# zssjh/stereo-semantic-vo

Measured on AMD Instinct MI355X. Metric: stereo frames/sec on KITTI 00 (full Tracking::Track chain), higher is better.
Workload: dtype u8; 1 GPU; BASELINE configs[2]: synth-kitti00 sequence of 4541 distinct 1241x376 stereo pairs, full Tracking::Track loop per frame (ORB on L and R, sparse stereo, matching passes 1+2, PnP-RANSAC, pose-only LM, map-point lifecycle); ONE sequence per GPU in strict frame order (replicas across GPUs); parallelism=one GPU, resident_pairs_per_gpu=4541, resident_input_bytes_per_gpu=4370984960, frames_tracked=4541, tracker_capacity_flag=0, pnp_samples_through_sequential_fallback=0

## Files before the change

stereo-semantic-vo_amd/csrc/svo_epnp_ord_dev.h:

```cpp
#pragma once
#ifndef HIP_INCLUDE_HIP_HIP_RUNTIME_H
#include <hip/hip_runtime.h>
#endif
#include <stdint.h>

#include "svo_epnp_exact_dev.h"

namespace epnp_ord {

#define EO_FN __device__ __forceinline__
typedef double d2 __attribute__((ext_vector_type(2)));

#include "svo_epnp_ord_tab.h"
#include "svo_epnp_ord_asm.h"

#define EO_SYNC()                                         \
  do {                                                    \
    __builtin_amdgcn_fence(__ATOMIC_ACQ_REL, "wavefront"); \
    __builtin_amdgcn_wave_barrier();                      \
  } while (0)

struct Lds {
  alignas(16) double jr[16 * 16];
  alignas(16) double xch[16][4][4];
  unsigned tab[EO_TAB_TOTAL];
  double pws[16], us[10], alphas[20], cws[12], ccinv[9];
  double M[120];
  double ut4[4][12];
  double L[60], rho[6];
  double sw[3][6];
  double bx[3][6];
  double ccs[3][12], pcs[3][16], abt[3][9], Rc[3][9], rep[3][8];
  alignas(16) double gn[3][6][6];
  double out[3][16];
  int srow[3][6];
  int urow[4];
  double xw[16];
  int flag;
  int sweeps;
  int why;
  long long stamp[8];
#ifdef EO_PROFILE
  long long prof[8];
#endif
};

EO_FN double xdiv(double a, double b) { return a / b; }
EO_FN double xsqrt(double x) { return sqrt(x); }

EO_FN double ndiv(double a, double b) {
  double r = __builtin_amdgcn_rcp(b);
  double e = __builtin_fma(-b, r, 1.0);
  r = __builtin_fma(r, e, r);
  e = __builtin_fma(-b, r, 1.0);
  r = __builtin_fma(r, e, r);
  const double q = a * r;
  const double rem = __builtin_fma(-b, q, a);
  return __builtin_fma(rem, r, q);
}
EO_FN double nsqrt(double x) {
  const double y = __builtin_amdgcn_rsq(x);
  double g = x * y, h = 0.5 * y;
  const double r = __builtin_fma(-h, g, 0.5);
  g = __builtin_fma(g, r, g);
  h = __builtin_fma(h, r, h);
  double d = __builtin_fma(-g, g, x);
  g = __builtin_fma(d, h, g);
  d = __builtin_fma(-g, g, x);
  g = __builtin_fma(d, h, g);
  return g;
}
EO_FN bool w_in_range(double w) { return w >= 7.888609052210118e-31 && w <= 1.2676506002282294e30; }

EO_FN double gsum(double term, double acc) { return __builtin_amdgcn_mfma_f64_4x4x4f64(1.0, term, acc, 0, 0, 0); }
template <int M>
EO_FN double colsum(double t0, double t1, double t2, int g) {
  double acc = gsum(M >= 4 || g < M ? t0 : 0.0, 0.0);
  if (M > 4) acc = gsum(M >= 8 || 4 + g < M ? t1 : 0.0, acc);
  if (M > 8) acc = gsum(M >= 12 || 8 + g < M ? t2 : 0.0, acc);
  return acc;
}

#define EO_TAB3_OFF 0
#define EO_TAB4_OFF (EO_TAB3_OFF + EO_TAB3_STEPS * 3)
#define EO_TAB5_OFF (EO_TAB4_OFF + EO_TAB4_STEPS * 4)
#define EO_TAB12_OFF (EO_TAB5_OFF + EO_TAB5_STEPS * 5)
EO_FN unsigned tab_entry(unsigned e) { return (e & ~16u) | ((e & 16u) << 27); }
EO_FN void load_tables(Lds& S, int lane) {
  for (int e = lane; e < EO_TAB3_STEPS * 3; e += 64) S.tab[EO_TAB3_OFF + e] = tab_entry(c_tab3[0][e]);
  for (int e = lane; e < EO_TAB4_STEPS * 4; e += 64) S.tab[EO_TAB4_OFF + e] = tab_entry(c_tab4[0][e]);
  for (int e = lane; e < EO_TAB5_STEPS * 5; e += 64) S.tab[EO_TAB5_OFF + e] = tab_entry(c_tab5[0][e]);
  for (int e = lane; e < EO_TAB12_STEPS * 12; e += 64) S.tab[EO_TAB12_OFF + e] = tab_entry(c_tab12[0][e]);
}

// ... 357 lines not shown
      double eta = fabs(A[k][k]);
#pragma unroll
      for (int i = k + 1; i < 6; ++i) {
        const double elt = fabs(A[i - 1][k]);
        if (eta < elt) eta = elt;
      }
      if (eta == 0) alive = false;
      const double inv_eta = 1. / eta;
      double sum2 = 0.0;
#pragma unroll
      for (int i = k; i < 6; ++i) {
        A[i][k] *= inv_eta;
        sum2 += A[i][k] * A[i][k];
      }
      double sigma = xsqrt(sum2);
      if (A[k][k] < 0) sigma = -sigma;
      A[k][k] += sigma;
      A1[k] = sigma * A[k][k];
      A2[k] = -eta * sigma;
#pragma unroll
      for (int j = k + 1; j < 4; ++j) {
        double sum = 0;
#pragma unroll
        for (int i = k; i < 6; ++i) sum += A[i][k] * A[i][j];
        const double tau = sum / A1[k];
#pragma unroll
        for (int i = k; i < 6; ++i) A[i][j] -= tau * A[i][k];
      }
    }
#pragma unroll
    for (int j = 0; j < 4; ++j) {
      double tau = 0;
#pragma unroll
      for (int i = j; i < 6; ++i) tau += A[i][j] * b[i];
      tau /= A1[j];
#pragma unroll
      for (int i = j; i < 6; ++i) b[i] -= tau * A[i][j];
    }
    x[3] = b[3] / A2[3];
#pragma unroll
    for (int i = 2; i >= 0; --i) {
      double sum = 0;
#pragma unroll
      for (int j = i + 1; j < 4; ++j) sum += A[i][j] * x[j];
      x[i] = (b[i] - sum) / A2[i];
    }
#pragma unroll
    for (int i = 0; i < 4; ++i) betas[i] += alive ? x[i] : 0.0;
  }
}

EO_FN double dot3(const double* a, const double* b) { return a[0] * b[0] + a[1] * b[1] + a[2] * b[2]; }

EO_FN bool solve5_wave(Lds& S, epnp_exact::Work& xw, const double* K, double* R_out, double* t_out, double* rep, bool force_seq = false) {
  const int lane = threadIdx.x & 63, slot = lane >> 4, col = lane & 15, r16 = lane & 15;
  const double fu = K[0], fv = K[1], uc = K[2], vc = K[3];
  if (lane == 0) { S.flag = force_seq ? 1 : 0; S.why = force_seq ? 16 : 0; S.stamp[0] = clock64(); }
  load_tables(S, lane);
  EO_SYNC();
  if (lane < 3) {
    double c = 0;
    for (int i = 0; i < 5; i++) c += S.pws[3 * i + lane];
    S.cws[lane] = c / 5;
  }
  EO_SYNC();
  auto load_pw0 = [&]() {
    if (lane < 9) {
      const int a = lane / 3, b = lane % 3;
      const double ca = S.cws[a], cb = S.cws[b];
      double s = 0;
      for (int i = 0; i < 5; ++i) s += (S.pws[3 * i + a] - ca) * (S.pws[3 * i + b] - cb);
      S.jr[b * 16 + a] = s;
    } else if (lane < 18) {
      const int r = (lane - 9) / 3, k = (lane - 9) % 3;
      S.jr[r * 16 + 3 + k] = r == k ? 1.0 : 0.0;
    } else if (lane < 36) {
      S.jr[((lane - 18) / 6) * 16 + 6 + (lane - 18) % 6] = 0.0;
    }
    EO_SYNC();
  };
  load_pw0();
  unsigned long long ex = jacobi_rows<3>(S, r16 < 3 ? 3 : 0, r16 < 3 ? 0 : r16, lane);
  unsigned long long bd = svd_rank(S, slot == 0 ? 3 : 0, 0, 0, lane);
  if (ex | bd) {
    load_pw0();
    if (lane == 0) svd_small_seq(S, xw.jW, 3, 3, 0, 0);
    EO_SYNC();
  }
  if (lane < 9) {
    const int i = 1 + lane / 3, j = lane % 3;
    const double k = xsqrt(S.sw[0][i - 1] / 5);
    S.cws[3 * i + j] = S.cws[j] + k * S.jr[S.srow[0][i - 1] * 16 + j];
  }
  EO_SYNC();
  auto load_cc = [&]() {
    if (lane < 9) {
      const int r = lane / 3, k = lane % 3;
      S.jr[r * 16 + k] = S.cws[3 * (r + 1) + k] - S.cws[k];
    } else if (lane < 18) {
      const int r = (lane - 9) / 3, k = (lane - 9) % 3;
      S.jr[r * 16 + 3 + k] = r == k ? 1.0 : 0.0;
    } else if (lane < 36) {
      S.jr[((lane - 18) / 6) * 16 + 6 + (lane - 18) % 6] = 0.0;
    }
    EO_SYNC();
  };
  load_cc();
  ex = jacobi_rows<3>(S, r16 < 3 ? 3 : 0, r16 < 3 ? 0 : r16, lane);
  bd = svd_rank(S, slot == 0 ? 3 : 0, 0, 0, lane);
  if (ex | bd) {
    load_cc();
    if (lane == 0) svd_small_seq(S, xw.jW, 3, 3, 0, 0);
// ... 271 lines not shown
```

stereo-semantic-vo_amd/csrc/svo_pose_dev.h:

```cpp
#pragma once
#include "svo_internal.h"
#include "svo_wave.h"

struct Se3 { double q[4]; double t[3]; };

__device__ __forceinline__ double pose_ndiv(double a, double b) {
  double r = __builtin_amdgcn_rcp(b);
  double e = __builtin_fma(-b, r, 1.0);
  r = __builtin_fma(r, e, r);
  e = __builtin_fma(-b, r, 1.0);
  r = __builtin_fma(r, e, r);
  const double q = a * r;
  const double rem = __builtin_fma(-b, q, a);
  return __builtin_fma(rem, r, q);
}
__device__ __forceinline__ double pose_rcp_refined(double b) {
  double r = __builtin_amdgcn_rcp(b);
  double e = __builtin_fma(-b, r, 1.0);
  r = __builtin_fma(r, e, r);
  e = __builtin_fma(-b, r, 1.0);
  r = __builtin_fma(r, e, r);
  return r;
}
__device__ __forceinline__ double pose_ndiv_r(double a, double b, double r) {
// ... 327 lines not shown

__device__ __forceinline__ void pose_edge_regs(const double* Xw, const double* obs, int n, double first[10], int sx = 3, int so = 2) {
  const int lane = threadIdx.x & 63, a = min(lane, n - 1), b = min(64 + lane, n - 1);
  first[0] = Xw[sx * a]; first[1] = Xw[sx * a + 1]; first[2] = Xw[sx * a + 2]; first[3] = obs[so * a]; first[4] = obs[so * a + 1];
  first[5] = Xw[sx * b]; first[6] = Xw[sx * b + 1]; first[7] = Xw[sx * b + 2]; first[8] = obs[so * b]; first[9] = obs[so * b + 1];
}

__device__ __forceinline__ void build_system_ordered(const Se3& est, const double* Xw, const double* obs, int n, const double* K,
                                                     double delta, double dsqr, double* tw_all , double* red,
                                                     bool on_mfma, const double first[10]) {
  const int tid = threadIdx.x, lane = tid & 63, wv = __builtin_amdgcn_readfirstlane(tid >> 6);
  const int g = lane >> 4, c = lane & 15;
  double* tw = tw_all + wv * POSE_CHUNK * POSE_TW;
  double acc = 0.0;
  for (int e0 = 0; e0 < n; e0 += POSE_CHUNK) {
    const int cnt = min(POSE_CHUNK, n - e0);
    if (cnt > 64) {
      switch (wv) {
        case 0: wave_terms_to_lds<0, true>(est, Xw, obs, n, e0, lane, K, delta, dsqr, tw, first); break;
        case 1: wave_terms_to_lds<1, true>(est, Xw, obs, n, e0, lane, K, delta, dsqr, tw, first); break;
        case 2: wave_terms_to_lds<2, true>(est, Xw, obs, n, e0, lane, K, delta, dsqr, tw, first); break;
        default: wave_terms_to_lds<3, true>(est, Xw, obs, n, e0, lane, K, delta, dsqr, tw, first); break;
      }
    } else {
      switch (wv) {
        case 0: wave_terms_to_lds<0, false>(est, Xw, obs, n, e0, lane, K, delta, dsqr, tw, first); break;
        case 1: wave_terms_to_lds<1, false>(est, Xw, obs, n, e0, lane, K, delta, dsqr, tw, first); break;
        case 2: wave_terms_to_lds<2, false>(est, Xw, obs, n, e0, lane, K, delta, dsqr, tw, first); break;
        default: wave_terms_to_lds<3, false>(est, Xw, obs, n, e0, lane, K, delta, dsqr, tw, first); break;
      }
    }
    POSE_WSYNC();
    if (on_mfma) acc = pose_chain_sum(tw + min(c, POSE_TW - 1), POSE_TW, cnt, g, acc);
    else acc = pose_lane_sum(tw + min(lane, POSE_QW - 1), POSE_TW, cnt, acc);
    POSE_WSYNC();
  }
  if (lane < POSE_QW) red[wv * POSE_QW + lane] = acc;
  __syncthreads();
}

__device__ __forceinline__ void unpack_system(const double* red, double H[36], double b[6]) {
  int k = 0;
#pragma unroll
  for (int r = 0; r < 6; ++r)
#pragma unroll
    for (int c = r; c < 6; ++c) { H[6 * r + c] = red[k]; H[6 * c + r] = red[k]; ++k; }
#pragma unroll
  for (int r = 0; r < 6; ++r) b[r] = red[21 + r];
}

struct LmShared {
  Se3 est;
  int go;
  int done;
};

#define PNP_HYP 100
#define PNP_MAXN 512

struct PoseLds {
  double tw[4 * POSE_CHUNK * POSE_TW];
  double red[POSE_NQ + 4];
  LmShared sh;
  double K[4];
};

__device__ __forceinline__ void build_system_one_lane(const Se3& est, const double* Xw, const double* obs, int n, const double* K,
                                                      double delta, double dsqr, double* red) {
  if (threadIdx.x == 0) {
    double acc[POSE_NQ];
    for (int k = 0; k < POSE_NQ; ++k) acc[k] = 0.0;
    for (int i = 0; i < n; ++i) {
      double e[2], pc[3], J[12], rz;
      edge_error(est, Xw + 3 * i, obs + 2 * i, K, e, pc, &rz);
      double rho0 = e[0] * e[0] + e[1] * e[1], rho1 = 1.;
      huber(rho0, delta, dsqr, rho0, rho1);
      edge_jacobian(pc, K, J, rz);
      int k = 0;
      for (int r = 0; r < 6; ++r)
        for (int c = r; c < 6; ++c) acc[k++] += rho1 * (J[r] * J[c] + J[6 + r] * J[6 + c]);
      for (int r = 0; r < 6; ++r) acc[21 + r] -= rho1 * (J[r] * e[0] + J[6 + r] * e[1]);
      acc[27] += rho0;
    }
    for (int k = 0; k < POSE_NQ; ++k) red[k] = acc[k];
  }
  __syncthreads();
}

struct PosePrepared { const Se3* est; const double* first; };
__device__ __forceinline__ void pose_start_estimate(const double* T, int round_in_f32, Se3& est0) {
  if (round_in_f32) {
    double Tf[16];
    for (int j = 0; j < 16; ++j) Tf[j] = (double)(float)T[j];
    se3_from_T(Tf, est0);
  } else {
    se3_from_T(T, est0);
  }
}

template <int NT = 256>
__device__ __forceinline__ void pose_opt_block(PoseLds& L, const double* __restrict__ Xw, const double* __restrict__ obs, int n,
                                               const double* __restrict__ Kp, double* T, svo_lm_stats* stats,
                                               int round_in_f32, int use_ordered_mfma, long long* t_first_build = nullptr,
                                               const PosePrepared* prep = nullptr, double* T_lds = nullptr, int* iters_out = nullptr) {
  static_assert(NT == 256, "pose_opt_block: four waves (wave w owns the quantities 7 w .. 7 w + 6 of the normal equations)");
  double* red = L.red; LmShared& sh = L.sh; double* K = L.K;
  const int tid = threadIdx.x;
  const double delta = (double)(float)sqrt(5.991);
  const double dsqr = delta * delta;
  Se3 est0{};
  double first[10];
  if (prep && prep->est) {
    if (tid == 0) { est0 = *prep->est; sh.est = est0; sh.done = 0; }
#pragma unroll
    for (int k = 0; k < 10; ++k) first[k] = prep->first[k];
  } else {
    __syncthreads();
    if (!prep && tid < 4) K[tid] = Kp[tid];
    if (tid == 0) {
      pose_start_estimate(T, round_in_f32, est0);
      sh.est = est0;
      sh.done = 0;
    }
    if (prep) {
#pragma unroll
      for (int k = 0; k < 10; ++k) first[k] = prep->first[k];
    } else if (n > 0) {
      pose_edge_regs(Xw, obs, n, first);
    }
  }
  __syncthreads();
  double lambda = -1., ni = 2., currentChi = 0, chi_init = 0;
  int nBad = 0, iters = 0, trials_total = 0, terminated = 0;
  if (n <= 0) {
    if (tid == 0 && stats) {
      stats->n_edges = 0; stats->iterations = 0; stats->trials_total = 0; stats->terminated = 0;
      stats->chi2_initial = 0; stats->chi2_final = 0; stats->lambda_final = 0;
    }
    if (tid == 0 && T_lds)
      for (int j = 0; j < 16; ++j) T_lds[j] = T[j];
    if (tid == 0 && iters_out) *iters_out = 0;
    return;
  }
#ifdef POSE_PROF
  long long pf_build = 0, pf_serial = 0, pf_dec = 0, pf_t = 0;
#define PF(acc) do { const long long _n = clock64(); acc += _n - pf_t; pf_t = _n; } while (0)
  pf_t = clock64();
#else
#define PF(acc) do { } while (0)
#endif
  auto build = [&]() {
    const Se3 est = sh.est;
    if (use_ordered_mfma) build_system_ordered(est, Xw, obs, n, K, delta, dsqr, L.tw, red, use_ordered_mfma == 1, first);
    else build_system_one_lane(est, Xw, obs, n, K, delta, dsqr, red);
  };
  if (t_first_build && tid == 0) *t_first_build = wall_clock64();
  build();
  PF(pf_build);
  double H[36], b[6], x[6] = {0, 0, 0, 0, 0, 0};
  if (tid == 0) {
    unpack_system(red, H, b);
    currentChi = red[27];
    chi_init = currentChi;
    double maxDiag = 0;
    for (int j = 0; j < 6; ++j) maxDiag = fmax(fabs(H[7 * j]), maxDiag);
    lambda = 1e-5 * maxDiag;
  }
  for (int it = 0; it < 10; ++it) {
    double iniChi = currentChi, rho = 0;
    int qmax = 0;
    for (int trial = 0; trial < 10; ++trial) {
      int ok2 = 0;
      if (tid == 0) {
        double Hl[36];
#pragma unroll
        for (int j = 0; j < 36; ++j) Hl[j] = H[j];
#pragma unroll
        for (int j = 0; j < 6; ++j) Hl[7 * j] += lambda;
        ok2 = ldlt6_solve(Hl, b, x);
        Se3 e2 = est0;
        se3_oplus(x, e2);
        sh.est = e2;
      }
      __syncthreads();
      PF(pf_serial);
      build();
      PF(pf_build);
      if (tid == 0) {
        double tempChi = red[27];
        if (!ok2) tempChi = 1.7976931348623157e308;
        rho = currentChi - tempChi;
        double scale = 0;
        for (int j = 0; j < 6; ++j) scale += x[j] * (lambda * x[j] + b[j]);
        scale += 1e-3;
        rho /= scale;
        if (rho > 0 && isfinite(tempChi)) {
          const double v = 2 * rho - 1;
          double alpha = 1. - v * v * v;
          alpha = fmin(alpha, 2. / 3.);
          const double scaleFactor = fmax(1. / 3., alpha);
          lambda *= scaleFactor;
          ni = 2;
          currentChi = tempChi;
          est0 = sh.est;
          unpack_system(red, H, b);
        } else {
          lambda *= ni;
          ni *= 2;
        }
        ++qmax;
        ++trials_total;
        sh.go = (rho < 0 && qmax < 10) ? 1 : 0;
      }
      __syncthreads();
      PF(pf_dec);
      if (!sh.go) break;
    }
    if (tid == 0) {
      ++iters;
      int stop = 0;
      if (qmax == 10 || rho == 0) stop = 1;
      else {
        if ((iniChi - currentChi) * 1e3 < iniChi) ++nBad; else nBad = 0;
        if (nBad >= 3) stop = 1;
      }
      if (stop) terminated = 1;
      sh.done = stop;
    }
    __syncthreads();
    if (sh.done) break;
  }
  if (tid == 0) {
    se3_to_T(est0, T);
    if (T_lds) se3_to_T(est0, T_lds);
    if (iters_out) *iters_out = iters;
    if (stats) {
      stats->n_edges = n; stats->iterations = iters; stats->trials_total = trials_total;
      stats->terminated = terminated; stats->chi2_initial = chi_init;
      stats->chi2_final = currentChi; stats->lambda_final = lambda;
#ifdef POSE_PROF
      stats->chi2_initial = (double)pf_build; stats->chi2_final = (double)pf_serial; stats->lambda_final = (double)pf_dec;
#endif
    }
  }
}

#include "svo_epnp_dev.h"
#include "svo_epnp_exact_dev.h"
#include "svo_epnp_ord_dev.h"

struct PnpHyp {
  double R[9], t[3];
  int32_t cnt, ok;
};

__device__ __forceinline__ bool pnp_inlier(const double* R, const double* t, const double* X, const double* uv, const double* K) {
  double x = R[0] * X[0] + R[1] * X[1] + R[2] * X[2] + t[0];
  double y = R[3] * X[0] + R[4] * X[1] + R[5] * X[2] + t[1];
  double z = R[6] * X[0] + R[7] * X[1] + R[8] * X[2] + t[2];
  z = z != 0.0 ? 1. / z : 1.;
  x *= z; y *= z;
  const float px = (float)(x * K[0] + K[2]), py = (float)(y * K[1] + K[3]);
  const float dx = (float)uv[0] - px, dy = (float)uv[1] - py;
  const float err = dx * dx + dy * dy;
  return err <= 64.0f;
}

__device__ __forceinline__ void pnp_hyp_block(EpnpWaveLds* ws, const double* Xw, const double* uv, int n, const double* K,
                                              const uint16_t* subset, PnpHyp* out, int hyp_base) {
  const int lane = threadIdx.x & 63, wv = threadIdx.x >> 6;
  const int k = hyp_base + wv;
  if (k >= PNP_HYP) return;
  if (lane < 5) {
    const int e = min((int)subset[5 * k + lane], n - 1);
    ws[wv].x5[3 * lane] = Xw[3 * e]; ws[wv].x5[3 * lane + 1] = Xw[3 * e + 1]; ws[wv].x5[3 * lane + 2] = Xw[3 * e + 2];
    ws[wv].u5[2 * lane] = uv[2 * e]; ws[wv].u5[2 * lane + 1] = uv[2 * e + 1];
  }
  double R[9], t[3];
  const bool ok = epnp5_wave(ws[wv], K, R, t);
  int cnt = 0;
  if (ok)
    for (int e = lane; e < n; e += 64) cnt += pnp_inlier(R, t, Xw + 3 * e, uv + 2 * e, K) ? 1 : 0;
  cnt = wave_sum_i32_dpp(cnt);
  if (lane == 0) {
    PnpHyp h;
#pragma unroll
    for (int i = 0; i < 9; ++i) h.R[i] = R[i];
    h.t[0] = t[0]; h.t[1] = t[1]; h.t[2] = t[2];
    h.cnt = cnt; h.ok = ok ? 1 : 0;
    out[k] = h;
  }
}

struct PnpExactLds { epnp_exact::Work W; double R[9], t[3]; int ok; };
__device__ __forceinline__ void pnp_hyp_exact_wave(PnpExactLds& S, const double* Xw, const double* uv, int n, const double* K,
                                                   const uint16_t* subset, PnpHyp* out, int k) {
  const int lane = threadIdx.x & 63;
  if (k >= PNP_HYP) return;
  if (lane == 0) {
    double* x5 = S.W.PW0;
    double* u5 = S.W.gA;
    for (int i = 0; i < 5; ++i) {
      const int e = min((int)subset[5 * k + i], n - 1);
      x5[3 * i] = Xw[3 * e]; x5[3 * i + 1] = Xw[3 * e + 1]; x5[3 * i + 2] = Xw[3 * e + 2];
      u5[2 * i] = uv[2 * e]; u5[2 * i + 1] = uv[2 * e + 1];
    }
    S.ok = epnp_exact::solve5(S.W, x5, u5, K, S.R, S.t, nullptr) ? 1 : 0;
  }
  __builtin_amdgcn_fence(__ATOMIC_ACQ_REL, "workgroup");
  __builtin_amdgcn_wave_barrier();
  double R[9], t[3];
#pragma unroll
  for (int i = 0; i < 9; ++i) R[i] = S.R[i];
#pragma unroll
  for (int i = 0; i < 3; ++i) t[i] = S.t[i];
  const bool ok = S.ok != 0;
  int cnt = 0;
  if (ok)
    for (int e = lane; e < n; e += 64) cnt += pnp_inlier(R, t, Xw + 3 * e, uv + 2 * e, K) ? 1 : 0;
  cnt = wave_sum_i32_dpp(cnt);
  if (lane == 0) {
    PnpHyp h;
#pragma unroll
    for (int i = 0; i < 9; ++i) h.R[i] = R[i];
    h.t[0] = t[0]; h.t[1] = t[1]; h.t[2] = t[2];
    h.cnt = cnt; h.ok = ok ? 1 : 0;
    out[k] = h;
  }
}

struct PnpOrdLds { epnp_ord::Lds S; epnp_exact::Work W; };
template <bool AGENT_OUT = false>
__device__ __forceinline__ void pnp_hyp_ord_wave(PnpOrdLds& L, const double* Xw, const double* uv, int n, const double* K,
                                                 const uint16_t* subset, PnpHyp* out, int k, bool force_seq = false,
                                                 unsigned* word = nullptr ) {
  const int lane = threadIdx.x & 63;
  if (k >= PNP_HYP) return;
  if (lane < 5) {
    const int e = min((int)subset[5 * k + lane], n - 1);
    L.S.pws[3 * lane] = Xw[3 * e]; L.S.pws[3 * lane + 1] = Xw[3 * e + 1]; L.S.pws[3 * lane + 2] = Xw[3 * e + 2];
    L.S.us[2 * lane] = uv[2 * e]; L.S.us[2 * lane + 1] = uv[2 * e + 1];
  }
  double R[9], t[3];
  const bool ok = epnp_ord::solve5_wave(L.S, L.W, K, R, t, nullptr, force_seq);
  int cnt = 0;
  if (ok)
    for (int e = lane; e < n; e += 64) cnt += pnp_inlier(R, t, Xw + 3 * e, uv + 2 * e, K) ? 1 : 0;
  cnt = wave_sum_i32_dpp(cnt);
  if (lane == 0) {
    if (word) *word = (ok ? 0x80000000u : 0u) | (unsigned)cnt;
    if (AGENT_OUT) {
      PnpHyp* o = out + k;
#pragma unroll
      for (int i = 0; i < 9; ++i) __hip_atomic_store(reinterpret_cast<long long*>(&o->R[i]), __builtin_bit_cast(long long, R[i]), __ATOMIC_RELAXED, __HIP_MEMORY_SCOPE_AGENT);
#pragma unroll
      for (int i = 0; i < 3; ++i) __hip_atomic_store(reinterpret_cast<long long*>(&o->t[i]), __builtin_bit_cast(long long, t[i]), __ATOMIC_RELAXED, __HIP_MEMORY_SCOPE_AGENT);
      __hip_atomic_store(&o->cnt, cnt, __ATOMIC_RELAXED, __HIP_MEMORY_SCOPE_AGENT);
      __hip_atomic_store(&o->ok, ok ? 1 : 0, __ATOMIC_RELAXED, __HIP_MEMORY_SCOPE_AGENT);
    } else {
      PnpHyp h;
#pragma unroll
      for (int i = 0; i < 9; ++i) h.R[i] = R[i];
      h.t[0] = t[0]; h.t[1] = t[1]; h.t[2] = t[2];
      h.cnt = cnt; h.ok = ok ? 1 : 0;
      out[k] = h;
    }
  }
}

__device__ __forceinline__ int pnp_update_iters(double ep, int maxIters) {
  const double p = 0.99;
  ep = fmax(ep, 0.); ep = fmin(ep, 1.);
  double num = fmax(1. - p, 2.2250738585072014e-308);
  double denom = 1. - pow(1. - ep, 5.0);
  if (denom < 2.2250738585072014e-308) return 0;
  num = log(num);
  denom = log(denom);
  return denom >= 0 || -num >= maxIters * (-denom) ? maxIters : (int)rint(num / denom);
}

__device__ __forceinline__ int pnp_bound_after(const int* cnt, const int* ok, int n, int m) {
  int niters = PNP_HYP, maxGood = 0;
  if (n == 5) return 1;
  for (int iter = 0; iter < m && iter < niters; ++iter) {
    if (!ok[iter]) continue;
    const int g = cnt[iter];
    if (g > max(maxGood, 4)) { maxGood = g; niters = pnp_update_iters((double)(n - g) / n, niters); }
  }
  return niters;
}

__device__ __forceinline__ void pnp_update_terms(int g, int n, double* ld, int* r) {
  double ep = (double)(n - g) / n;
  ep = fmax(ep, 0.); ep = fmin(ep, 1.);
  const double denom = 1. - pow(1. - ep, 5.0);
  if (denom < 2.2250738585072014e-308) { *ld = 1.0; *r = 0; return; }
  const double num = log(fmax(1. - 0.99, 2.2250738585072014e-308));
  *ld = log(denom);
  *r = *ld < 0 ? (int)rint(num / *ld) : 0;
}
__device__ __forceinline__ int pnp_select_pre(const int* cnt, const int* ok, const double* ld, const int* r, int n, int* good, int* iters) {
  int niters = PNP_HYP, maxGood = 0, best = -1, run = 0;
  if (n == 5) {
    *good = ok[0] ? 5 : 0; *iters = 1;
    return ok[0] ? 0 : -1;
  }
  const double num = log(fmax(1. - 0.99, 2.2250738585072014e-308));
  for (int iter = 0; iter < niters; ++iter) {
    ++run;
// ... 75 lines not shown
```

stereo-semantic-vo_amd/csrc/svo_track.hip:

```cpp
#include <chrono>
#include <cstddef>
#include <initializer_list>
#include <string>
#include <vector>
#include <algorithm>
#include <cstring>
#include <mutex>

#include "svo_internal.h"
#include "svo_wave.h"
#include "svo_gate.h"
#include "svo_pose_dev.h"
#include "svo_fmat_dev.h"

#define TRK_MAXKP 512
#define TRK_CAP 4096
#define TRK_ROWS_MAX 3072
#define TRK_LCAP 8
#define TRK_GPOS (1 << 20)
#define TRK_DNC 24
#define TRK_DENSE 0xFF

struct TrackPool {
  alignas(16) uint32_t desc[TRK_CAP * 8];
  int32_t create_id[TRK_CAP];
  int32_t gid[TRK_CAP];
  uint8_t bad[TRK_CAP];
  uint8_t in_local[TRK_CAP];
};

#define TP_EARLY 8
#define TP_FLAGS 16
struct TrackWork {
  int32_t ready;
  int32_t frame_id, nkp, n_stereo, n_pass1, n_pass2, n_new, n_local, skip_match;
  long long ts[8];
  long long rt[6];
  int32_t diag[2];
  int32_t n_edges;
  int32_t edge_gid[TRK_MAXKP];
  int32_t edge_kp[TRK_MAXKP];
  int32_t new_gid[TRK_MAXKP];
  int32_t pnp_best, pnp_iterations, pnp_inliers, pnp_ok;
  double T_pnp[16];
  int32_t hyp_done, pad_hyp;
  long long hyp_early[TP_FLAGS];
  long long hyp_rt[TP_EARLY];
};

struct TrackState {
  int32_t frame_num, npool, lastN, cur;
  int32_t next_gid, overflow, n_vetoed, n_boxes;
  int32_t epnp_fallbacks, pad_counters[3];
  int32_t last_mp[TRK_MAXKP];
  int32_t dbg_cur_mp[TRK_MAXKP];
  svo_camera cam;
  int32_t boxes[SVO_MAX_BOXES * 4];
  double F[9];
  float last_xy[TRK_MAXKP * 2];
  alignas(16) uint32_t last_desc[TRK_MAXKP * 8];
  int32_t bf_idx[TRK_MAXKP], bf_dist[TRK_MAXKP], bf_min;
  uint8_t bf_keep[TRK_MAXKP];
  float lastTcw[16];
  double Xw[TRK_MAXKP * 3], obs[TRK_MAXKP * 2], K[4], Tprior[16], T[16];
  svo_lm_stats lm;
  svo_pnp_stats pnp;
  PnpHyp hyp[PNP_HYP];
  long long pose_ts[16];
  TrackPool pool[2];
  uint16_t rowmin[TRK_CAP];
  uint8_t ncand[TRK_CAP];
  uint32_t cand[(size_t)TRK_CAP * 2 * TRK_LCAP];
  uint16_t D[(size_t)TRK_CAP * 512];
  float gpos[(size_t)TRK_GPOS * 3];
};

__device__ __forceinline__ int tk_wave_incl_scan(int v) {
  v += __builtin_amdgcn_update_dpp(0, v, 0x111, 0xf, 0xf, false);
  v += __builtin_amdgcn_update_dpp(0, v, 0x112, 0xf, 0xf, false);
  v += __builtin_amdgcn_update_dpp(0, v, 0x114, 0xf, 0xf, false);
  v += __builtin_amdgcn_update_dpp(0, v, 0x118, 0xf, 0xf, false);
  v += __builtin_amdgcn_update_dpp(0, v, 0x142, 0xa, 0xf, false);
  v += __builtin_amdgcn_update_dpp(0, v, 0x143, 0xc, 0xf, false);
  return v;
}
__device__ __forceinline__ int block_excl_scan(int v, int* sm , int* total) {
  const int lane = threadIdx.x & 63, wv = threadIdx.x >> 6;
  const int incl = tk_wave_incl_scan(v);
  const int nw = blockDim.x >> 6;
  __syncthreads();
  if (lane == 63) sm[wv] = incl;
  __syncthreads();
  const int4 a = reinterpret_cast<const int4*>(sm)[0], b = reinterpret_cast<const int4*>(sm)[1],
             c = reinterpret_cast<const int4*>(sm)[2], d = reinterpret_cast<const int4*>(sm)[3];
  const int t[16] = {a.x, a.y, a.z, a.w, b.x, b.y, b.z, b.w, c.x, c.y, c.z, c.w, d.x, d.y, d.z, d.w};
  int off = 0, tot = 0;
#pragma unroll
  for (int w = 0; w < 16; ++w) {
    off += w < wv ? t[w] : 0;
    tot += w < nw ? t[w] : 0;
  }
  *total = tot;
  return off + incl - v;
}

__device__ __forceinline__ void tk_unproject(const svo_camera& cam, float u, float v, float z,
                                             const float* Rwc, const float* twc, float* xyz) {
  const float x = (u - cam.cx) * z * (1 / cam.fx);
  const float y = (v - cam.cy) * z * (1 / cam.fy);
#pragma unroll
  for (int r = 0; r < 3; ++r) {
    const double acc = (double)Rwc[3 * r] * (double)x + (double)Rwc[3 * r + 1] * (double)y +
                       (double)Rwc[3 * r + 2] * (double)z;
    xyz[r] = (float)(acc + (double)twc[r]);
  }
}

__device__ __forceinline__ int ld_agent(const int* p) { return __hip_atomic_load(p, __ATOMIC_RELAXED, __HIP_MEMORY_SCOPE_AGENT); }
__device__ __forceinline__ long long ld_agent(const long long* p) { return __hip_atomic_load(p, __ATOMIC_RELAXED, __HIP_MEMORY_SCOPE_AGENT); }
__device__ __forceinline__ void st_agent(int* p, int v) { __hip_atomic_store(p, v, __ATOMIC_RELAXED, __HIP_MEMORY_SCOPE_AGENT); }
__device__ __forceinline__ void st_agent(long long* p, long long v) { __hip_atomic_store(p, v, __ATOMIC_RELAXED, __HIP_MEMORY_SCOPE_AGENT); }
// ... 800 lines not shown
    if ((int)threadIdx.x < pre) { S.cnt[threadIdx.x] = st->hyp[threadIdx.x].cnt; S.ok[threadIdx.x] = st->hyp[threadIdx.x].ok; }
    __syncthreads();
    if (threadIdx.x == 0) S.bound = pnp_bound_after(S.cnt, S.ok, n, pre);
    __syncthreads();
    if (first >= S.bound) return;
  }
  const float* gpos = st->gpos;
  for (int e = threadIdx.x; e < n; e += blockDim.x) {
    const bool first_e = e == (int)threadIdx.x;
    const float* gp = gpos + 3 * (size_t)((first_e ? gid0 : ld_agent(&work->edge_gid[e])) & (TRK_GPOS - 1));
    const svo_kp k = kp[first_e ? j0 : ld_agent(&work->edge_kp[e])];
    S.Xw[3 * e] = (double)gp[0]; S.Xw[3 * e + 1] = (double)gp[1]; S.Xw[3 * e + 2] = (double)gp[2];
    S.uv[2 * e] = (double)k.x; S.uv[2 * e + 1] = (double)k.y;
  }
  __syncthreads();
  const double K[4] = {(double)st->cam.fx, (double)st->cam.fy, (double)st->cam.cx, (double)st->cam.cy};
  const long long t_gather = clock64();
  pnp_hyp_block(S.ws, S.Xw, S.uv, n, K, subsets + (size_t)min(n, 512) * 500, st->hyp, first);
  if (first == 0 && threadIdx.x == 0) {
    st->pose_ts[0] = t_start; st->pose_ts[1] = t_gather; st->pose_ts[2] = S.ws[0].stamp[0]; st->pose_ts[3] = S.ws[0].stamp[4];
    st->pose_ts[4] = clock64();
    st->pose_ts[5] = S.ws[0].stamp[1]; st->pose_ts[6] = S.ws[0].stamp[2]; st->pose_ts[7] = S.ws[0].stamp[3]; st->pose_ts[12] = S.ws[0].sweeps;
    st->pose_ts[13] = S.ws[0].stamp[5]; st->pose_ts[14] = S.ws[0].stamp[6]; st->pose_ts[15] = S.ws[0].stamp[7];
  }
}

struct TpHypExactLds { double Xw[TRK_MAXKP * 3], uv[TRK_MAXKP * 2]; PnpExactLds ex; };
__global__ __launch_bounds__(64) void k_tp_hyp_exact(TrackState* st, TrackWork* work, const svo_kp* kp, const uint16_t* subsets,
                                                     int kstride, int tag) {
  TpHypExactLds& S = *reinterpret_cast<TpHypExactLds*>(tk_smem);
  st += blockIdx.y; work += blockIdx.y; kp += (size_t)blockIdx.y * kstride;
  if (!tp_wait_work(st, work, tag)) return;
  if (threadIdx.x == 0 && blockIdx.x == 0) work->rt[2] = wall_clock64();
  const int n = ld_agent(&work->n_edges);
  if (ld_agent(&work->skip_match) || n < 5) return;
  const float* gpos = st->gpos;
  for (int e = threadIdx.x; e < n; e += blockDim.x) {
    const float* gp = gpos + 3 * (size_t)(ld_agent(&work->edge_gid[e]) & (TRK_GPOS - 1));
    const svo_kp k = kp[ld_agent(&work->edge_kp[e])];
    S.Xw[3 * e] = (double)gp[0]; S.Xw[3 * e + 1] = (double)gp[1]; S.Xw[3 * e + 2] = (double)gp[2];
    S.uv[2 * e] = (double)k.x; S.uv[2 * e + 1] = (double)k.y;
  }
  __syncthreads();
  const double K[4] = {(double)st->cam.fx, (double)st->cam.fy, (double)st->cam.cx, (double)st->cam.cy};
  pnp_hyp_exact_wave(S.ex, S.Xw, S.uv, n, K, subsets + (size_t)min(n, 512) * 500, st->hyp, blockIdx.x);
}

struct TpHypOrdLds { double Xw[TRK_MAXKP * 3], uv[TRK_MAXKP * 2]; PnpOrdLds ord; int cnt[TP_HYP_PRE], ok[TP_HYP_PRE], bound; };
template <bool FUSED>
__device__ __forceinline__ void tp_hyp_ord_body(TpHypOrdLds& S, TrackState* st, TrackWork* work, const svo_kp* kp, const uint16_t* subsets,
                                                int kstride, int hyp_base, int sample, int tag, int force_seq, int semi = 0) {
  if (!tp_wait_work(st, work, tag)) return;
  const long long t_start = clock64();
  if (threadIdx.x == 0 && sample == 0) work->rt[2] = wall_clock64();
  const int n = ld_agent(&work->n_edges);
  const int frame_tag = FUSED ? ld_agent(&work->frame_id) + 1 : 0;
  if (ld_agent(&work->skip_match) || n < 5) return;
  if (FUSED && (force_seq >> 8) == sample + 1) return;
  if (FUSED && semi > 0) {
    const int tid = threadIdx.x;
    if (tid < semi) { S.cnt[tid] = ld_agent(&st->hyp[tid].cnt); S.ok[tid] = ld_agent(&st->hyp[tid].ok); }
    __syncthreads();
    if (tid == 0) S.bound = pnp_bound_after(S.cnt, S.ok, n, semi);
    __syncthreads();
    bool leave = sample >= S.bound;
    if (!leave && sample >= 2 * semi) {
      if (tid >= semi && tid < 2 * semi) {
        int spins = 0;
        long long w = 0;
        while (tp_early_tag(w = ld_agent(&work->hyp_early[tid])) != frame_tag && spins < (1 << 22)) { __builtin_amdgcn_s_sleep(2); ++spins; }
        const bool late = spins >= (1 << 22);
        S.cnt[tid] = late ? 0 : tp_early_cnt(w); S.ok[tid] = late ? 0 : tp_early_ok(w);
      }
      __syncthreads();
      if (tid == 0) S.bound = pnp_bound_after(S.cnt, S.ok, n, 2 * semi);
      __syncthreads();
      leave = sample >= S.bound;
    }
    if (leave) {
      if (tid == 0) {
        if (sample < TP_FLAGS) st_agent(&work->hyp_early[sample], tp_early_word(frame_tag, 0u));
        __hip_atomic_fetch_add(&work->hyp_done, 1, __ATOMIC_RELAXED, __HIP_MEMORY_SCOPE_AGENT);
      }
      return;
    }
  }
  if (hyp_base > 0) {
    const int pre = min(hyp_base, TP_HYP_PRE);
    if ((int)threadIdx.x < pre) { S.cnt[threadIdx.x] = st->hyp[threadIdx.x].cnt; S.ok[threadIdx.x] = st->hyp[threadIdx.x].ok; }
    __syncthreads();
    if (threadIdx.x == 0) S.bound = pnp_bound_after(S.cnt, S.ok, n, pre);
    __syncthreads();
    if (sample >= S.bound) return;
  }
  const float* gpos = st->gpos;
  for (int e = threadIdx.x; e < n; e += 64) {
    const float* gp = gpos + 3 * (size_t)(ld_agent(&work->edge_gid[e]) & (TRK_GPOS - 1));
    const svo_kp k = kp[ld_agent(&work->edge_kp[e])];
    S.Xw[3 * e] = (double)gp[0]; S.Xw[3 * e + 1] = (double)gp[1]; S.Xw[3 * e + 2] = (double)gp[2];
    S.uv[2 * e] = (double)k.x; S.uv[2 * e + 1] = (double)k.y;
  }
  __syncthreads();
  const double K[4] = {(double)st->cam.fx, (double)st->cam.fy, (double)st->cam.cx, (double)st->cam.cy};
  if (!FUSED && sample == 0) {
    for (int i = threadIdx.x; i < 3 * n; i += 64) st->Xw[i] = S.Xw[i];
    for (int i = threadIdx.x; i < 2 * n; i += 64) st->obs[i] = S.uv[i];
    if (threadIdx.x < 4) st->K[threadIdx.x] = K[threadIdx.x];
  }
  const long long t_gather = clock64();
  unsigned ok_cnt = 0;
  pnp_hyp_ord_wave<FUSED>(S.ord, S.Xw, S.uv, n, K, subsets + (size_t)min(n, 512) * 500, st->hyp, sample, (force_seq & 0xff) != 0, &ok_cnt);
  if (FUSED) {
    if (threadIdx.x == 0 && sample < TP_EARLY) st_agent(&work->hyp_rt[sample], (long long)wall_clock64());
    TP_STORES_DONE();
    if (threadIdx.x == 0) {
      if (sample < TP_FLAGS) st_agent(&work->hyp_early[sample], tp_early_word(frame_tag, ok_cnt));
      __hip_atomic_fetch_add(&work->hyp_done, 1, __ATOMIC_RELAXED, __HIP_MEMORY_SCOPE_AGENT);
    }
  }
  if (threadIdx.x == 0 && S.ord.S.flag) atomicAdd(&st->epnp_fallbacks, 1);
  if (sample == 0 && threadIdx.x == 0) {
    const long long* sp = S.ord.S.stamp;
    st->pose_ts[0] = t_start; st->pose_ts[1] = t_gather; st->pose_ts[2] = sp[0]; st->pose_ts[3] = sp[7];
    st->pose_ts[4] = clock64();
    st->pose_ts[5] = sp[2]; st->pose_ts[6] = sp[3]; st->pose_ts[7] = sp[4]; st->pose_ts[12] = S.ord.S.flag;
    st->pose_ts[13] = sp[4]; st->pose_ts[14] = sp[5]; st->pose_ts[15] = sp[6];
  }
}
__global__ __launch_bounds__(64) void k_tp_hyp_ord(TrackState* st, TrackWork* work, const svo_kp* kp, const uint16_t* subsets,
                                                   int kstride, int hyp_base, int tag, int force_seq) {
  TpHypOrdLds& S = *reinterpret_cast<TpHypOrdLds*>(tk_smem);
  st += blockIdx.y; work += blockIdx.y; kp += (size_t)blockIdx.y * kstride;
  tp_hyp_ord_body<false>(S, st, work, kp, subsets, kstride, hyp_base, hyp_base + (int)blockIdx.x, tag, force_seq);
}
__global__ __launch_bounds__(64) void k_tp_hyp_ord_first(TrackState* st, TrackWork* work, const svo_kp* kp, const uint16_t* subsets,
                                                         int kstride, int tag, int force_seq) {
  TpHypOrdLds& S = *reinterpret_cast<TpHypOrdLds*>(tk_smem);
  st += blockIdx.y; work += blockIdx.y; kp += (size_t)blockIdx.y * kstride;
  tp_hyp_ord_body<true>(S, st, work, kp, subsets, kstride, 0, (int)blockIdx.x, tag, force_seq);
}

struct TpLds {
  PoseLds pose;
  alignas(16) int sm[16];
  int cnt[PNP_HYP], ok[PNP_HYP], upd_r[PNP_HYP], best, good, iters;
  long long hrt[TP_EARLY];
  double tab_ld[PNP_MAXN + 1]; int tab_r[PNP_MAXN + 1];
  double pre_T[TP_EARLY][16]; Se3 pre_est[TP_EARLY];
  double T_end[16];
  long long t_samples, t_build;
  int late[TP_EARLY], lost;
  int recf[8];
  double upd_ld[PNP_HYP];
};

#define TPF_NT 256
template <bool FUSED>
__device__ __forceinline__ void tp_frame_body(TpLds& S, TrackState* st, TrackWork* work, const svo_kp* kp, const float* depth,
                                              svo_track_result* res_out, int kstride, int use_mfma, int tag, int pre_gathered) {
  const int tid = threadIdx.x;
  if (!tp_wait_work(st, work, tag)) return;
  if (!FUSED && tid == 0) work->rt[4] = wall_clock64();
  const long long tf0 = clock64();
  const int id = ld_agent(&work->frame_id), nkp = ld_agent(&work->nkp), skip = ld_agent(&work->skip_match), n_edges = ld_agent(&work->n_edges);
  const int gid0 = ld_agent(&work->edge_gid[tid]), j0 = min(max(ld_agent(&work->edge_kp[tid]), 0), kstride - 1);
  float* gpos = st->gpos;
  if (tid >= 64 && tid < 71) {
    const int* src = tid == 64 ? &work->n_stereo : tid == 65 ? &work->n_pass1 : tid == 66 ? &work->n_pass2 : tid == 67 ? &work->n_new
                   : tid == 68 ? &work->n_local : tid == 69 ? &work->diag[0] : &work->diag[1];
    S.recf[tid - 64] = ld_agent(src);
  }
  constexpr int NEWS = (TRK_MAXKP + TPF_NT - 1) / TPF_NT;
  int new_g[NEWS]; svo_kp new_k[NEWS]; float new_d[NEWS];
#pragma unroll
  for (int q = 0; q < NEWS; ++q) {
    const int j = tid + q * TPF_NT;
    new_g[q] = ld_agent(&work->new_gid[min(j, TRK_MAXKP - 1)]);
    new_k[q] = kp[min(j, kstride - 1)];
    new_d[q] = depth[min(j, kstride - 1)];
// ... 1318 lines not shown
      SVO_HIP(c0, pull(sg->depth + r0 * K, c->d_depth + (size_t)f0 * K, wf * b));
      SVO_HIP(c0, pull(sg->n + r0, c->d_nkp + f0, 4 * (size_t)b));
    }
    if (!any) break;
    SVO_HIP(c0, hipEventRecord(sg->ev_sub[j], sg->gs));
    if (sub_off[j] * G < B) wait[(size_t)sub_off[j] * G] = sg->ev_sub[j];
  }
  SVO_HIP(c0, hipEventRecord(sg->ev_gathered, sg->gs));
  sg->row_of_frame.resize(B);
  for (int k = 0; k < B; ++k) sg->row_of_frame[k] = (int)set0 + (k % G) * rper + k / G;
  rc = tail_enqueue(c0, sg->kp, sg->desc, sg->n, sg->depth, K, B, 1, d_results, boxes, wait.data(), sg->row_of_frame.data(), p,
                    nullptr, true);
  if (rc) return rc;
  SVO_HIP(c0, hipEventRecord(sg->done[p], c0->stream));
  for (int g = 0; g < G; ++g) {
    ctxs[g]->shard_wait = sg->ev_gathered;
    if (std::find(sg->producers.begin(), sg->producers.end(), ctxs[g]) == sg->producers.end()) sg->producers.push_back(ctxs[g]);
  }
  sg->used[p] = true;
  sg->parity ^= 1;
  c0->track_frame += B;
  return SVO_OK;
}

extern "C" int svo_track_sharded_dev(svo_ctx* const* ctxs, int G, const uint8_t* const* d_grayL, const uint8_t* const* d_grayR,
                                     int stride, int B, const svo_boxes_dev* boxes, svo_track_result* d_results) {
  return svo_track_sharded_fed(ctxs, G, d_grayL, d_grayR, stride, B, boxes, d_results, nullptr);
}

extern "C" int svo_debug_track_pnp(svo_ctx* ctx, svo_pnp_stats* stats, double T_pnp[16]) {
  if (!ctx || !ctx->d_track) return SVO_E_INVALID;
  TrackState* st = reinterpret_cast<TrackState*>(ctx->d_track);
  SVO_HIP(ctx, hipStreamSynchronize(ctx->stream));
  if (stats) SVO_HIP(ctx, svo_memcpy_sync(ctx, stats, &st->pnp, sizeof *stats, hipMemcpyDeviceToHost));
  if (T_pnp) {
    PnpHyp h;
    svo_pnp_stats s;
    SVO_HIP(ctx, svo_memcpy_sync(ctx, &s, &st->pnp, sizeof s, hipMemcpyDeviceToHost));
    if (s.best_hypothesis < 0) return SVO_E_INVALID;
    SVO_HIP(ctx, svo_memcpy_sync(ctx, &h, &st->hyp[s.best_hypothesis], sizeof h, hipMemcpyDeviceToHost));
    for (int r = 0; r < 3; ++r) { for (int c = 0; c < 3; ++c) T_pnp[4 * r + c] = h.R[3 * r + c]; T_pnp[4 * r + 3] = h.t[r]; }
    T_pnp[12] = 0; T_pnp[13] = 0; T_pnp[14] = 0; T_pnp[15] = 1;
  }
  return SVO_OK;
}

extern "C" int svo_debug_track_pose_stamps(svo_ctx* ctx, int64_t ts[16]) {
  if (!ctx || !ts || !ctx->d_track) return SVO_E_INVALID;
  SVO_HIP(ctx, hipStreamSynchronize(ctx->stream));
  TrackState* st = reinterpret_cast<TrackState*>(ctx->d_track);
  SVO_HIP(ctx, svo_memcpy_sync(ctx, ts, st->pose_ts, sizeof(long long) * 16, hipMemcpyDeviceToHost));
  return SVO_OK;
}
```

Measured before the change: 9974 stereo frames/s.

## Overlap PnP hypothesis gathers and table loads with work wait; merge LM barriers

The PnP hypothesis kernel now loads the EPnP tables and prefetches the first 128 edge indices, camera intrinsics and subset indices before checking skip, so these loads overlap the latency of the work hand-off. The sample's five correspondence indices are passed in directly, and solve5_wave skips its own table load when tables are already present. Hypothesis R/t stores are issued right after the solve instead of after inlier counting. In pose-only LM, the per-iteration termination decision is folded into the trial-decision barrier, removing one __syncthreads per iteration. It also adds extra timestamp probes and a debug export. The cost is extra speculative loads even when the frame is skipped.

New measurement: 10060 stereo frames/s, median of 6. About the same (+0.9%).

```diff
diff --git a/stereo-semantic-vo_amd/csrc/svo_epnp_ord_dev.h b/stereo-semantic-vo_amd/csrc/svo_epnp_ord_dev.h
--- a/stereo-semantic-vo_amd/csrc/svo_epnp_ord_dev.h
+++ b/stereo-semantic-vo_amd/csrc/svo_epnp_ord_dev.h
@@ -39,7 +39,7 @@
   int flag;
   int sweeps;
   int why;
-  long long stamp[8];
+  long long stamp[9];
 #ifdef EO_PROFILE
   long long prof[8];
 #endif
@@ -503,12 +503,14 @@
 
 EO_FN double dot3(const double* a, const double* b) { return a[0] * b[0] + a[1] * b[1] + a[2] * b[2]; }
 
-EO_FN bool solve5_wave(Lds& S, epnp_exact::Work& xw, const double* K, double* R_out, double* t_out, double* rep, bool force_seq = false) {
+EO_FN bool solve5_wave(Lds& S, epnp_exact::Work& xw, const double* K, double* R_out, double* t_out, double* rep, bool force_seq = false,
+                       bool tables_loaded = false) {
   const int lane = threadIdx.x & 63, slot = lane >> 4, col = lane & 15, r16 = lane & 15;
   const double fu = K[0], fv = K[1], uc = K[2], vc = K[3];
   if (lane == 0) { S.flag = force_seq ? 1 : 0; S.why = force_seq ? 16 : 0; S.stamp[0] = clock64(); }
-  load_tables(S, lane);
-  EO_SYNC();
+  if (!tables_loaded) load_tables(S, lane);
+  EO_SYNC();
+  if (lane == 0) S.stamp[8] = clock64();
   if (lane < 3) {
     double c = 0;
     for (int i = 0; i < 5; i++) c += S.pws[3 * i + lane];
diff --git a/stereo-semantic-vo_amd/csrc/svo_pose_dev.h b/stereo-semantic-vo_amd/csrc/svo_pose_dev.h
--- a/stereo-semantic-vo_amd/csrc/svo_pose_dev.h
+++ b/stereo-semantic-vo_amd/csrc/svo_pose_dev.h
@@ -403,7 +403,6 @@
 struct LmShared {
   Se3 est;
   int go;
-  int done;
 };
 
 #define PNP_HYP 100
@@ -462,7 +461,7 @@
   Se3 est0{};
   double first[10];
   if (prep && prep->est) {
-    if (tid == 0) { est0 = *prep->est; sh.est = est0; sh.done = 0; }
+    if (tid == 0) { est0 = *prep->est; sh.est = est0; }
 #pragma unroll
     for (int k = 0; k < 10; ++k) first[k] = prep->first[k];
   } else {
@@ -471,7 +470,6 @@
     if (tid == 0) {
       pose_start_estimate(T, round_in_f32, est0);
       sh.est = est0;
-      sh.done = 0;
     }
     if (prep) {
 #pragma unroll
@@ -494,11 +492,13 @@
     return;
   }
 #ifdef POSE_PROF
-  long long pf_build = 0, pf_serial = 0, pf_dec = 0, pf_t = 0;
+  long long pf_build = 0, pf_serial = 0, pf_dec = 0, pf_t = 0, pf_bar = 0;
 #define PF(acc) do { const long long _n = clock64(); acc += _n - pf_t; pf_t = _n; } while (0)
+#define PF_BARRIER() do { const long long _b = clock64(); __syncthreads(); pf_bar += clock64() - _b; } while (0)
   pf_t = clock64();
 #else
 #define PF(acc) do { } while (0)
+#define PF_BARRIER() __syncthreads()
 #endif
   auto build = [&]() {
     const Se3 est = sh.est;
@@ -519,7 +519,7 @@
   }
   for (int it = 0; it < 10; ++it) {
     double iniChi = currentChi, rho = 0;
-    int qmax = 0;
+    int qmax = 0, verdict = 0;
     for (int trial = 0; trial < 10; ++trial) {
       int ok2 = 0;
       if (tid == 0) {
@@ -533,7 +533,7 @@
         se3_oplus(x, e2);
         sh.est = e2;
       }
-      __syncthreads();
+      PF_BARRIER();
       PF(pf_serial);
       build();
       PF(pf_build);
@@ -561,25 +561,25 @@
         }
         ++qmax;
         ++trials_total;
-        sh.go = (rho < 0 && qmax < 10) ? 1 : 0;
+        const int go = (rho < 0 && qmax < 10) ? 1 : 0;
+        int stop = 0;
+        if (!go) {
+          ++iters;
+          if (qmax == 10 || rho == 0) stop = 1;
+          else {
+            if ((iniChi - currentChi) * 1e3 < iniChi) ++nBad; else nBad = 0;
+            if (nBad >= 3) stop = 1;
+          }
+          if (stop) terminated = 1;
+        }
+        sh.go = go | (stop << 1);
       }
-      __syncthreads();
+      PF_BARRIER();
       PF(pf_dec);
-      if (!sh.go) break;
-    }
-    if (tid == 0) {
-      ++iters;
-      int stop = 0;
-      if (qmax == 10 || rho == 0) stop = 1;
-      else {
-        if ((iniChi - currentChi) * 1e3 < iniChi) ++nBad; else nBad = 0;
-        if (nBad >= 3) stop = 1;
-      }
-      if (stop) terminated = 1;
-      sh.done = stop;
-    }
-    __syncthreads();
-    if (sh.done) break;
+      verdict = sh.go;
+      if (!(verdict & 1)) break;
+    }
+    if (verdict & 2) break;
   }
   if (tid == 0) {
     se3_to_T(est0, T);
@@ -591,6 +591,7 @@
       stats->chi2_final = currentChi; stats->lambda_final = lambda;
 #ifdef POSE_PROF
       stats->chi2_initial = (double)pf_build; stats->chi2_final = (double)pf_serial; stats->lambda_final = (double)pf_dec;
+      stats->terminated = (int)pf_bar;
 #endif
     }
   }
@@ -684,16 +685,26 @@
 template <bool AGENT_OUT = false>
 __device__ __forceinline__ void pnp_hyp_ord_wave(PnpOrdLds& L, const double* Xw, const double* uv, int n, const double* K,
                                                  const uint16_t* subset, PnpHyp* out, int k, bool force_seq = false,
-                                                 unsigned* word = nullptr ) {
+                                                 int e5 = -1 ,
+                                                 unsigned* word = nullptr ,
+                                                 long long* rt_out = nullptr ) {
   const int lane = threadIdx.x & 63;
   if (k >= PNP_HYP) return;
   if (lane < 5) {
-    const int e = min((int)subset[5 * k + lane], n - 1);
+    const int e = min(e5 >= 0 ? e5 : (int)subset[5 * k + lane], n - 1);
     L.S.pws[3 * lane] = Xw[3 * e]; L.S.pws[3 * lane + 1] = Xw[3 * e + 1]; L.S.pws[3 * lane + 2] = Xw[3 * e + 2];
     L.S.us[2 * lane] = uv[2 * e]; L.S.us[2 * lane + 1] = uv[2 * e + 1];
   }
   double R[9], t[3];
-  const bool ok = epnp_ord::solve5_wave(L.S, L.W, K, R, t, nullptr, force_seq);
+  const bool ok = epnp_ord::solve5_wave(L.S, L.W, K, R, t, nullptr, force_seq, e5 >= 0);
+  if (AGENT_OUT && lane == 0) {
+    PnpHyp* o = out + k;
+#pragma unroll
+    for (int i = 0; i < 9; ++i) __hip_atomic_store(reinterpret_cast<long long*>(&o->R[i]), __builtin_bit_cast(long long, R[i]), __ATOMIC_RELAXED, __HIP_MEMORY_SCOPE_AGENT);
+#pragma unroll
+    for (int i = 0; i < 3; ++i) __hip_atomic_store(reinterpret_cast<long long*>(&o->t[i]), __builtin_bit_cast(long long, t[i]), __ATOMIC_RELAXED, __HIP_MEMORY_SCOPE_AGENT);
+    if (rt_out) __hip_atomic_store(rt_out, (long long)wall_clock64(), __ATOMIC_RELAXED, __HIP_MEMORY_SCOPE_AGENT);
+  }
   int cnt = 0;
   if (ok)
     for (int e = lane; e < n; e += 64) cnt += pnp_inlier(R, t, Xw + 3 * e, uv + 2 * e, K) ? 1 : 0;
@@ -702,10 +713,6 @@
     if (word) *word = (ok ? 0x80000000u : 0u) | (unsigned)cnt;
     if (AGENT_OUT) {
       PnpHyp* o = out + k;
-#pragma unroll
-      for (int i = 0; i < 9; ++i) __hip_atomic_store(reinterpret_cast<long long*>(&o->R[i]), __builtin_bit_cast(long long, R[i]), __ATOMIC_RELAXED, __HIP_MEMORY_SCOPE_AGENT);
-#pragma unroll
-      for (int i = 0; i < 3; ++i) __hip_atomic_store(reinterpret_cast<long long*>(&o->t[i]), __builtin_bit_cast(long long, t[i]), __ATOMIC_RELAXED, __HIP_MEMORY_SCOPE_AGENT);
       __hip_atomic_store(&o->cnt, cnt, __ATOMIC_RELAXED, __HIP_MEMORY_SCOPE_AGENT);
       __hip_atomic_store(&o->ok, ok ? 1 : 0, __ATOMIC_RELAXED, __HIP_MEMORY_SCOPE_AGENT);
     } else {
diff --git a/stereo-semantic-vo_amd/csrc/svo_track.hip b/stereo-semantic-vo_amd/csrc/svo_track.hip
--- a/stereo-semantic-vo_amd/csrc/svo_track.hip
+++ b/stereo-semantic-vo_amd/csrc/svo_track.hip
@@ -66,7 +66,7 @@
   svo_lm_stats lm;
   svo_pnp_stats pnp;
   PnpHyp hyp[PNP_HYP];
-  long long pose_ts[16];
+  long long pose_ts[24];
   TrackPool pool[2];
   uint16_t rowmin[TRK_CAP];
   uint8_t ncand[TRK_CAP];
@@ -973,10 +973,20 @@
                                                 int kstride, int hyp_base, int sample, int tag, int force_seq, int semi = 0) {
   if (!tp_wait_work(st, work, tag)) return;
   const long long t_start = clock64();
-  if (threadIdx.x == 0 && sample == 0) work->rt[2] = wall_clock64();
+  const long long w_start = wall_clock64();
   const int n = ld_agent(&work->n_edges);
   const int frame_tag = FUSED ? ld_agent(&work->frame_id) + 1 : 0;
-  if (ld_agent(&work->skip_match) || n < 5) return;
+  const int skip0 = ld_agent(&work->skip_match);
+  int gid2[2], j2[2];
+#pragma unroll
+  for (int q = 0; q < 2; ++q) {
+    gid2[q] = ld_agent(&work->edge_gid[threadIdx.x + 64 * q]) & (TRK_GPOS - 1);
+    j2[q] = min(max(ld_agent(&work->edge_kp[threadIdx.x + 64 * q]), 0), kstride - 1);
+  }
+  const svo_camera cam = st->cam;
+  epnp_ord::load_tables(S.ord.S, threadIdx.x);
+  if (threadIdx.x == 0 && sample == 0) work->rt[2] = w_start;
+  if (skip0 || n < 5) return;
   if (FUSED && (force_seq >> 8) == sample + 1) return;
   if (FUSED && semi > 0) {
     const int tid = threadIdx.x;
@@ -1015,14 +1025,32 @@
     if (sample >= S.bound) return;
   }
   const float* gpos = st->gpos;
-  for (int e = threadIdx.x; e < n; e += 64) {
+  const uint16_t* subset_row = subsets + (size_t)min(n, 512) * 500;
+  float gx[2][3], kx[2][2];
+#pragma unroll
+  for (int q = 0; q < 2; ++q) {
+    const float* gp = gpos + 3 * (size_t)gid2[q];
+    const svo_kp* k = kp + j2[q];
+    gx[q][0] = gp[0]; gx[q][1] = gp[1]; gx[q][2] = gp[2];
+    kx[q][0] = k->x; kx[q][1] = k->y;
+  }
+  const int e5 = threadIdx.x < 5 ? (int)subset_row[5 * sample + threadIdx.x] : 0;
+#pragma unroll
+  for (int q = 0; q < 2; ++q) {
+    const int e = threadIdx.x + 64 * q;
+    if (e < n) {
+      S.Xw[3 * e] = (double)gx[q][0]; S.Xw[3 * e + 1] = (double)gx[q][1]; S.Xw[3 * e + 2] = (double)gx[q][2];
+      S.uv[2 * e] = (double)kx[q][0]; S.uv[2 * e + 1] = (double)kx[q][1];
+    }
+  }
+  for (int e = threadIdx.x + 128; e < n; e += 64) {
     const float* gp = gpos + 3 * (size_t)(ld_agent(&work->edge_gid[e]) & (TRK_GPOS - 1));
     const svo_kp k = kp[ld_agent(&work->edge_kp[e])];
     S.Xw[3 * e] = (double)gp[0]; S.Xw[3 * e + 1] = (double)gp[1]; S.Xw[3 * e + 2] = (double)gp[2];
     S.uv[2 * e] = (double)k.x; S.uv[2 * e + 1] = (double)k.y;
   }
   __syncthreads();
-  const double K[4] = {(double)st->cam.fx, (double)st->cam.fy, (double)st->cam.cx, (double)st->cam.cy};
+  const double K[4] = {(double)cam.fx, (double)cam.fy, (double)cam.cx, (double)cam.cy};
   if (!FUSED && sample == 0) {
     for (int i = threadIdx.x; i < 3 * n; i += 64) st->Xw[i] = S.Xw[i];
     for (int i = threadIdx.x; i < 2 * n; i += 64) st->obs[i] = S.uv[i];
@@ -1030,10 +1058,13 @@
   }
   const long long t_gather = clock64();
   unsigned ok_cnt = 0;
-  pnp_hyp_ord_wave<FUSED>(S.ord, S.Xw, S.uv, n, K, subsets + (size_t)min(n, 512) * 500, st->hyp, sample, (force_seq & 0xff) != 0, &ok_cnt);
+  pnp_hyp_ord_wave<FUSED>(S.ord, S.Xw, S.uv, n, K, subset_row, st->hyp, sample, (force_seq & 0xff) != 0, e5, &ok_cnt,
+                          (FUSED && sample < TP_EARLY) ? &work->hyp_rt[sample] : nullptr);
+  const long long t_counted = clock64();
+  long long t_drained = t_counted;
   if (FUSED) {
-    if (threadIdx.x == 0 && sample < TP_EARLY) st_agent(&work->hyp_rt[sample], (long long)wall_clock64());
     TP_STORES_DONE();
+    t_drained = clock64();
     if (threadIdx.x == 0) {
       if (sample < TP_FLAGS) st_agent(&work->hyp_early[sample], tp_early_word(frame_tag, ok_cnt));
       __hip_atomic_fetch_add(&work->hyp_done, 1, __ATOMIC_RELAXED, __HIP_MEMORY_SCOPE_AGENT);
@@ -1046,6 +1077,7 @@
     st->pose_ts[4] = clock64();
     st->pose_ts[5] = sp[2]; st->pose_ts[6] = sp[3]; st->pose_ts[7] = sp[4]; st->pose_ts[12] = S.ord.S.flag;
     st->pose_ts[13] = sp[4]; st->pose_ts[14] = sp[5]; st->pose_ts[15] = sp[6];
+    st->pose_ts[16] = sp[8]; st->pose_ts[17] = t_counted; st->pose_ts[18] = t_drained;
   }
 }
 __global__ __launch_bounds__(64) void k_tp_hyp_ord(TrackState* st, TrackWork* work, const svo_kp* kp, const uint16_t* subsets,
@@ -2470,3 +2502,10 @@
   SVO_HIP(ctx, svo_memcpy_sync(ctx, ts, st->pose_ts, sizeof(long long) * 16, hipMemcpyDeviceToHost));
   return SVO_OK;
 }
+extern "C" int svo_debug_track_pose_stamps_ext(svo_ctx* ctx, int64_t ts[24]) {
+  if (!ctx || !ts || !ctx->d_track) return SVO_E_INVALID;
+  SVO_HIP(ctx, hipStreamSynchronize(ctx->stream));
+  TrackState* st = reinterpret_cast<TrackState*>(ctx->d_track);
+  SVO_HIP(ctx, svo_memcpy_sync(ctx, ts, st->pose_ts, sizeof(long long) * 24, hipMemcpyDeviceToHost));
+  return SVO_OK;
+}
```
